# 3dv-casia/PanoVLM

Hardware: AMD Instinct MI355X
Metric: M residual+Jacobian evals/sec (point-to-plane, 64k pts/scan) (higher is better)
Workload: dtype f64

## Files before the change

panovlm_amd/csrc/pvlm_eval.hip:

```cpp
#include <algorithm>
#include <cmath>
#include <limits>

#include "pvlm_functors.h"
#include "pvlm_internal.h"

using namespace pvlm_dev;

#ifndef PVLM_NT_LOADS
#define PVLM_NT_LOADS 1
#endif
#ifndef PVLM_GLOBAL_LOADS
#define PVLM_GLOBAL_LOADS 1
#endif
typedef double pvlm_dbl2 __attribute__((ext_vector_type(2)));
#if PVLM_GLOBAL_LOADS
template <class T> using pvlm_gptr = const __attribute__((address_space(1))) T*;
#else
template <class T> using pvlm_gptr = const T*;
#endif
typedef pvlm_gptr<pvlm_dbl2> pvlm_col_ptr;
#ifndef PVLM_NT_LOADS_MATERIALISE
#define PVLM_NT_LOADS_MATERIALISE 0
#endif
__device__ __forceinline__ const double* at_byte(const double* base, unsigned bytes) {
  return reinterpret_cast<const double*>(reinterpret_cast<const char*>(base) + bytes);
}
template <bool NT>
__device__ __forceinline__ double2 stream_load2(const double* p) {
  pvlm_col_ptr q = (pvlm_col_ptr)(p);
  const pvlm_dbl2 v = NT ? __builtin_nontemporal_load(q) : *q;
  return make_double2(v.x, v.y);
}
struct pvlm_plane_args {
  const uint16_t* idx;
  const int64_t* pair_idx0;
  const int64_t* chunk_plane0;
  const double* tab;
  const double* const* pair_ptab;
  const int* order;
};
template <bool NT>
__device__ __forceinline__ unsigned stream_load_runs(const uint16_t* base, unsigned row) {
  const auto q = (pvlm_gptr<unsigned>)(reinterpret_cast<const char*>(base) + 2u * row);
  return NT ? __builtin_nontemporal_load(q) : *q;
}
template <bool NT>
__device__ __forceinline__ double stream_load1(const double* p) {
  const auto q = (pvlm_gptr<double>)(p);
  return NT ? __builtin_nontemporal_load(q) : *q;
}
template <bool NT>
__device__ __forceinline__ unsigned stream_load_run(const uint16_t* base, unsigned bytes) {
  const auto q = (pvlm_gptr<uint16_t>)(reinterpret_cast<const char*>(base) + (bytes >> 2));
  return NT ? __builtin_nontemporal_load(q) : *q;
}
template <bool NT>
__device__ __forceinline__ unsigned stream_load_word(const uint16_t* base, unsigned bytes) {
  const auto q = (pvlm_gptr<unsigned>)(reinterpret_cast<const char*>(base) + (bytes >> 1));
  return NT ? __builtin_nontemporal_load(q) : *q;
}
__device__ __forceinline__ double table_load(const double* base, unsigned bytes) {
  return *(pvlm_gptr<double>)(reinterpret_cast<const char*>(base) + bytes);
}
#ifndef PVLM_NT_STORES
#define PVLM_NT_STORES 0
#endif
__device__ __forceinline__ void stream_store2(double2* p, double2 v) {
#if PVLM_NT_STORES
  pvlm_dbl2 w; w.x = v.x; w.y = v.y;
  __builtin_nontemporal_store(w, reinterpret_cast<pvlm_dbl2*>(p));
#else
  *p = v;
#endif
}
__device__ __forceinline__ void stream_store1(double* p, double v) {
#if PVLM_NT_STORES
  __builtin_nontemporal_store(v, p);
#else
  *p = v;
#endif
}


#if defined(__HIP_DEVICE_COMPILE__)
#define PVLM_SCHED_FENCE() __builtin_amdgcn_sched_barrier(0)
#else
#define PVLM_SCHED_FENCE() ((void)0)
#endif
#ifndef PVLM_PREFETCH
#define PVLM_PREFETCH -1
#endif
#ifndef PVLM_FUSED_WAVES
#define PVLM_FUSED_WAVES 2
#endif
#ifndef PVLM_FUSED_WAVES_7COL
#define PVLM_FUSED_WAVES_7COL 4
#endif
#ifndef PVLM_FUSED_WAVES_WAVEFORM
#define PVLM_FUSED_WAVES_WAVEFORM 3
#endif

__global__ void k_pose_table(int n, const double* __restrict__ aa, const double* __restrict__ t, double* __restrict__ tab) {
  const int i = blockIdx.x * blockDim.x + threadIdx.x;
  if (i >= n) return;
  const double x = aa[3 * i], y = aa[3 * i + 1], z = aa[3 * i + 2];
  const double th2 = x * x + y * y + z * z;
  double* o = tab + (size_t)i * PVLM_POSE_TAB;
  double R[9];
  if (th2 > 2.220446049250313e-16) {
    const double th = sqrt(th2);
    const double wx = x / th, wy = y / th, wz = z / th;
    const double c = cos(th), s = sin(th), k = 1.0 - c;
    R[0] = c + wx * wx * k;      R[1] = wx * wy * k - wz * s; R[2] = wy * s + wx * wz * k;
    R[3] = wz * s + wx * wy * k; R[4] = c + wy * wy * k;      R[5] = -wx * s + wy * wz * k;
    R[6] = -wy * s + wx * wz * k; R[7] = wx * s + wy * wz * k; R[8] = c + wz * wz * k;
  } else {
    R[0] = 1; R[1] = -z; R[2] = y; R[3] = z; R[4] = 1; R[5] = -x; R[6] = -y; R[7] = x; R[8] = 1;
  }
  double A, B;
  if (th2 > 1e-6) {
    const double th = sqrt(th2);
    A = (1.0 - cos(th)) / th2;
    B = (th - sin(th)) / (th2 * th);
  } else {
    A = 0.5 - th2 * (1.0 / 24.0) + th2 * th2 * (1.0 / 720.0);
    B = (1.0 / 6.0) - th2 * (1.0 / 120.0) + th2 * th2 * (1.0 / 5040.0);
  }
  const double J[9] = {1.0 + B * (x * x - th2), -A * z + B * x * y,       A * y + B * x * z,
                       A * z + B * x * y,       1.0 + B * (y * y - th2), -A * x + B * y * z,
                       -A * y + B * x * z,      A * x + B * y * z,        1.0 + B * (z * z - th2)};
#pragma unroll
  for (int k = 0; k < 9; ++k) { o[k] = R[k]; o[9 + k] = J[k]; }
  o[18] = t[3 * i]; o[19] = t[3 * i + 1]; o[20] = t[3 * i + 2];
}

__global__ void k_pair_table(int P, const int* __restrict__ ref, const int* __restrict__ nei, int n_poses,
                             const double* __restrict__ pose, double* __restrict__ tab) {
  const int p = blockIdx.x * blockDim.x + threadIdx.x;
  if (p >= P) return;
  const int ir = ref[p], in = nei[p];
  double* o = tab + (size_t)p * PVLM_PAIR_TAB;
  if (ir >= n_poses || in >= n_poses) {
    for (int k = 0; k < PVLM_PAIR_TAB; ++k) o[k] = __longlong_as_double(0x7ff8000000000000LL);
    return;
  }
  const double* a = pose + (size_t)ir * PVLM_POSE_TAB;
  const double* b = pose + (size_t)in * PVLM_POSE_TAB;
  double R[9];
#pragma unroll
  for (int i = 0; i < 3; ++i)
#pragma unroll
    for (int j = 0; j < 3; ++j) R[i * 3 + j] = a[i * 3] * b[j * 3] + a[i * 3 + 1] * b[j * 3 + 1] + a[i * 3 + 2] * b[j * 3 + 2];
#pragma unroll
  for (int k = 0; k < 9; ++k) o[k] = R[k];
#pragma unroll
  for (int i = 0; i < 3; ++i) {
    o[9 + i] = a[18 + i] - (R[i * 3] * b[18] + R[i * 3 + 1] * b[19] + R[i * 3 + 2] * b[20]);
    o[12 + i] = a[18 + i];
  }
#pragma unroll
  for (int k = 0; k < 9; ++k) o[15 + k] = a[9 + k];
#pragma unroll
  for (int i = 0; i < 3; ++i)
#pragma unroll
    for (int j = 0; j < 3; ++j) o[24 + i * 3 + j] = -(R[i * 3] * b[9 + j] + R[i * 3 + 1] * b[9 + 3 + j] + R[i * 3 + 2] * b[9 + 6 + j]);
}

struct pvlm_segment {
  int p;
  const double* cols;
  int64_t n_dev;
  int64_t o0;
  int64_t lo, hi;
};
__device__ __forceinline__ pvlm_segment load_segment(int entry, const double* const* __restrict__ pair_cols, const int64_t* __restrict__ pair_stride,
                                                     const int64_t* __restrict__ out_start, const int* __restrict__ blk_pair,
                                                     const int* __restrict__ blk_chunk, int chunk_rows, int64_t row0 = 0) {
  pvlm_segment s;
  s.p = blk_pair[entry];
  s.cols = pair_cols[s.p];
  s.n_dev = pair_stride[s.p];
  s.o0 = out_start[s.p] - row0;
  const int64_t len = out_start[s.p + 1] - out_start[s.p];
  s.lo = (int64_t)blk_chunk[entry] * chunk_rows;
  s.hi = min(len, s.lo + (int64_t)chunk_rows);
  return s;
}

template <int KIND, bool NORM, int NCOLS>
__global__ __launch_bounds__(256) void k_eval_materialise(const double* const* __restrict__ pair_cols,
                                                          const int64_t* __restrict__ pair_stride,
                                                          const int64_t* __restrict__ out_start,
                                                          const int* __restrict__ blk_pair, const int* __restrict__ blk_chunk,
                                                          int chunk_rows, const double* __restrict__ pair_tab, double weight,
                                                          double* __restrict__ r_out, double* __restrict__ J_out, int blk0, int64_t row0) {
  const auto [p, cols, n_dev, o0, lo, hi] = load_segment(blockIdx.x + blk0, pair_cols, pair_stride, out_start, blk_pair, blk_chunk, chunk_rows, row0);
  double T[PVLM_PAIR_TAB];
#pragma unroll
  for (int k = 0; k < PVLM_PAIR_TAB; ++k) T[k] = pair_tab[(size_t)p * PVLM_PAIR_TAB + k];
  __shared__ __attribute__((aligned(16))) double stage[4][128 * 12];
  const int lane = threadIdx.x & 63, wv = threadIdx.x >> 6;
  const double* Jl = T + 15; const double* Mn = T + 24; const double* R = T;
  const int64_t n_it = (hi - lo + 511) / 512;
  for (int64_t it = 0; it < n_it; ++it) {
    const int64_t j = lo + it * 512 + 2 * (int64_t)threadIdx.x;
    if (j < hi) {
      double2 v[NCOLS];
#pragma unroll
      for (int c = 0; c < NCOLS; ++c) v[c] = stream_load2<PVLM_NT_LOADS_MATERIALISE != 0>(cols + (size_t)c * n_dev + j);
#pragma unroll
      for (int h = 0; h < 2; ++h) {
        if (j + h >= hi) break;
        double rec[NCOLS];
#pragma unroll
        for (int c = 0; c < NCOLS; ++c) rec[c] = h ? v[c].y : v[c].x;
        Wrench w;
        eval_wrench<KIND, NORM>(rec, T, weight, w);
        stream_store1(r_out + o0 + j + h, w.r);
        if (J_out) {
          double Jr[12];
#pragma unroll
          for (int k = 0; k < 3; ++k) {
            Jr[k] = w.c[0] * Jl[k] + w.c[1] * Jl[3 + k] + w.c[2] * Jl[6 + k];
            Jr[3 + k] = w.g[k];
            Jr[6 + k] = w.c[0] * Mn[k] + w.c[1] * Mn[3 + k] + w.c[2] * Mn[6 + k];
            Jr[9 + k] = -(w.g[0] * R[k] + w.g[1] * R[3 + k] + w.g[2] * R[6 + k]);
          }
          double2* dst = reinterpret_cast<double2*>(&stage[wv][(2 * lane + h) * 12]);
#pragma unroll
          for (int k = 0; k < 6; ++k) dst[k] = make_double2(Jr[2 * k], Jr[2 * k + 1]);
        }
      }
    }
    if (J_out) {
      __builtin_amdgcn_wave_barrier();
      const int64_t row0 = lo + it * 512 + (int64_t)wv * 128;
      const int64_t rows = min((int64_t)128, hi - row0);
      if (rows > 0) {
        double2* gdst = reinterpret_cast<double2*>(J_out + (size_t)(o0 + row0) * 12);
        const double2* src = reinterpret_cast<const double2*>(&stage[wv][0]);
        const int n2 = (int)rows * 6;
#pragma unroll
        for (int t = 0; t < 12; ++t) {
          const int e = t * 64 + lane;
          if (e < n2) stream_store2(gdst + e, src[e]);
        }
      }
      __builtin_amdgcn_wave_barrier();
    }
  }
}

template <int KIND, bool NORM, int NCOLS, int W>
__global__ __launch_bounds__(256) void k_eval_wrench(const double* const* __restrict__ pair_cols, const int64_t* __restrict__ pair_stride,
                                                     const int64_t* __restrict__ out_start, const int* __restrict__ blk_pair,
                                                     const int* __restrict__ blk_chunk, int chunk_rows, const double* __restrict__ pair_tab,
                                                     double weight, double* __restrict__ w_out, int blk0, int64_t row0) {
  const auto [p, cols, n_dev, o0, lo, hi] = load_segment(blockIdx.x + blk0, pair_cols, pair_stride, out_start, blk_pair, blk_chunk, chunk_rows, row0);
  double T[15];
#pragma unroll
  for (int k = 0; k < 15; ++k) T[k] = pair_tab[(size_t)p * PVLM_PAIR_TAB + k];
  __shared__ double stage[4][128 * W];
  const int lane = threadIdx.x & 63, wv = threadIdx.x >> 6;
  const int64_t n_it = (hi - lo + 511) / 512;
  for (int64_t it = 0; it < n_it; ++it) {
    const int64_t j = lo + it * 512 + 2 * (int64_t)threadIdx.x;
    if (j < hi) {
      double2 v[NCOLS];
#pragma unroll
      for (int c = 0; c < NCOLS; ++c) v[c] = stream_load2<PVLM_NT_LOADS_MATERIALISE != 0>(cols + (size_t)c * n_dev + j);
#pragma unroll
      for (int h = 0; h < 2; ++h) {
        if (j + h >= hi) break;
        double rec[NCOLS];
#pragma unroll
        for (int c = 0; c < NCOLS; ++c) rec[c] = h ? v[c].y : v[c].x;
        Wrench w;
        eval_wrench<KIND, NORM>(rec, T, weight, w);
        double* dst = &stage[wv][(2 * lane + h) * W];
        if (W == 7) { dst[0] = w.r; dst[1] = w.c[0]; dst[2] = w.c[1]; dst[3] = w.c[2]; dst[4] = w.g[0]; dst[5] = w.g[1]; dst[6] = w.g[2]; }
        else { dst[0] = w.r; dst[1] = w.g[0]; dst[2] = w.g[1]; dst[3] = w.g[2]; }
      }
    }
    __builtin_amdgcn_wave_barrier();
    const int64_t r0 = lo + it * 512 + (int64_t)wv * 128;
    const int64_t rows = min((int64_t)128, hi - r0);
    if (rows > 0) {
      double* g = w_out + (size_t)(o0 + r0) * W;
      const int n = (int)rows * W;
#pragma unroll
      for (int t = 0; t < 2 * W; ++t) {
        const int e = t * 64 + lane;
        if (e < n) stream_store1(g + e, stage[wv][e]);
      }
    }
    __builtin_amdgcn_wave_barrier();
  }
}

__device__ __forceinline__ double wave_sum(double x) {
#pragma unroll
  for (int off = 32; off > 0; off >>= 1) x += __shfl_down(x, off, 64);
  return x;
}

#ifndef PVLM_HUBER_SLOT
#define PVLM_HUBER_SLOT 1
#endif

template <bool WEIGHTED>
__device__ __forceinline__ void accumulate_outer(const double (&vv)[6], double r, double rho1, double half_rho, double* acc) {
  int q = 0;
#pragma unroll
  for (int a = 0; a < 6; ++a) {
    const double wa = WEIGHTED ? rho1 * vv[a] : vv[a];
#pragma unroll
    for (int b = a; b < 6; ++b, ++q) acc[q] = fma(wa, vv[b], acc[q]);
    acc[21 + a] = fma(wa, r, acc[21 + a]);
  }
  acc[27] += half_rho;
}

template <int KIND, bool NORM, int NCOLS, int LOSS>
__device__ __forceinline__ void accumulate_row(const double* rec, const double* T, double weight, double loss_a, double a2, double mh_a2, double* acc) {
  Wrench w;
  eval_wrench<KIND, NORM>(rec, T, weight, w);
  const double s = w.r * w.r;
  const double vv[6] = {w.c[0], w.c[1], w.c[2], w.g[0], w.g[1], w.g[2]};
  if (LOSS != PVLM_LOSS_HUBER) { accumulate_outer<false>(vv, w.r, 1.0, 0.5 * s, acc); return; }
  const bool out = s > a2;
  auto general = [&]() {
    const double rr = fabs(w.r);
    const double inv = fast_rcp(out ? rr : 1.0);
    const double rho1 = out ? fmax(std::numeric_limits<double>::min(), loss_a * inv) : 1.0;
    const double half_rho = out ? fma(loss_a, rr, mh_a2) : 0.5 * s;
    accumulate_outer<true>(vv, w.r, rho1, half_rho, acc);
  };
#if PVLM_HUBER_SLOT && defined(__HIP_DEVICE_COMPILE__)
  const unsigned long long outliers = __ballot(out);
  unsigned long long none = outliers;
  asm("" : "+s"(none));
  if (outliers != 0) general();
  if (none == 0) accumulate_outer<false>(vv, w.r, 1.0, 0.5 * s, acc);
#else
  general();
#endif
}

template <int N>
__device__ __forceinline__ double wave_transpose_sum(const double (&a)[N], int lane) {
  static_assert(N <= 32, "at most 32 values");
  double v[32];
#pragma unroll
  for (int k = 0; k < 32; ++k) v[k] = k < N ? a[k] : 0.0;
#pragma unroll
  for (int half = 16; half >= 1; half >>= 1) {
    const bool up = (lane & (2 * half)) != 0;
#pragma unroll
    for (int k = 0; k < half; ++k) {
      const double keep = up ? v[half + k] : v[k];
      const double send = up ? v[k] : v[half + k];
      v[k] = keep + __shfl_xor(send, 2 * half, 64);
    }
  }
  return v[0] + __shfl_xor(v[0], 1, 64);
}

template <int KIND, bool NORM, int NCOLS, int LOSS, bool PR, bool PT, bool ROT>
__global__ __launch_bounds__(256, (NCOLS == 7 ? PVLM_FUSED_WAVES_7COL : PVLM_FUSED_WAVES)) void k_eval_fused(const double* const* __restrict__ pair_cols,
                                                    const int64_t* __restrict__ pair_stride,
                                                    const int64_t* __restrict__ out_start,
                                                    const int* __restrict__ blk_pair, const int* __restrict__ blk_chunk,
                                                    int chunk_rows, const double* __restrict__ pair_tab, double weight,
                                                    double loss_a, double* __restrict__ partials, pvlm_plane_args pr) {
  static_assert(!PR || NCOLS == 7, "plane runs: the 7-column kinds only");
  static_assert(!PT || PR, "the point table: on top of the plane runs only");
  static_assert(!ROT || PR, "rotated halves: the plane-run forms only");
  const int slot = (PT && pr.order) ? pr.order[blockIdx.x] : (int)blockIdx.x;
  if (PT && slot < 0) return;
  constexpr int NS = PR ? 3 : NCOLS;
  const auto [p, cols, n_dev, o0, lo, hi] = load_segment(slot, pair_cols, pair_stride, out_start, blk_pair, blk_chunk, chunk_rows);
  double T[15];
#pragma unroll
  for (int k = 0; k < 15; ++k) T[k] = pair_tab[(size_t)p * PVLM_PAIR_TAB + k];
  double acc[PVLM_PARTIAL];
#pragma unroll
  for (int k = 0; k < PVLM_PARTIAL; ++k) acc[k] = 0.0;
  const double a2 = uniform_sgpr(loss_a * loss_a), mh_a2 = uniform_sgpr(-0.5 * a2);
  constexpr bool kRotate = ROT;
  constexpr bool kPrefetch = !PR && (PVLM_PREFETCH >= 0 ? (PVLM_PREFETCH != 0) : (KIND == PVLM_POINT2PLANE_METER || KIND == PVLM_POINT2LINE_METER));
  const double* colb[NS];
#pragma unroll
  for (int c = 0; c < NS; ++c) colb[c] = PT ? pr.pair_ptab[p] + (size_t)c * PVLM_POINT_TAB_STRIDE : cols + (size_t)c * n_dev + lo;
  const uint16_t* runb = nullptr;
  const double* tabb = nullptr;
  if (PR) { runb = pr.idx + (PT ? 2 : 1) * (pr.pair_idx0[p] + lo); tabb = pr.tab + 4 * pr.chunk_plane0[slot]; }
  const unsigned span = hi > lo ? (unsigned)(hi - lo) : 0u;
  const unsigned span8 = 8u * span, last8 = span8 - 8u;
  unsigned o = 8u * (threadIdx.x + (threadIdx.x & ~63u));
  auto row_at = [&](unsigned bytes) { return min(bytes, last8); };
  double x[2][NS], nx[2][NS];
  double2 pl[2][2];
  unsigned w[2] = {0u, 0u};
  auto load_word = [&](int h, unsigned bytes) {
    if (PT) w[h] = stream_load_word<PVLM_NT_LOADS != 0>(runb, bytes);
    else w[h] = stream_load_run<PVLM_NT_LOADS != 0>(runb, bytes);
  };
  auto load_cols = [&](double (&dst)[NS], unsigned bytes) {
#pragma unroll
    for (int c = 0; c < NS; ++c) dst[c] = stream_load1<PVLM_NT_LOADS != 0>(at_byte(colb[c], bytes));
  };
  auto gather = [&](int h, unsigned bytes) {
    if (PT) {
      const unsigned q = 8u * (w[h] >> 16);
#pragma unroll
      for (int c = 0; c < NS; ++c) x[h][c] = table_load(colb[c], q);
    } else {
      load_cols(x[h], bytes);
    }
    if (PR) {
      const unsigned at = 32u * (w[h] & 0xffffu);
      pl[h][0] = stream_load2<false>(at_byte(tabb, at));
      pl[h][1] = stream_load2<false>(at_byte(tabb, at + 16u));
      PVLM_SCHED_FENCE();
    }
  };
  auto evaluate = [&](int h, unsigned bytes) {
    if (bytes < span8) {
      double rec[NCOLS];
#pragma unroll
      for (int c = 0; c < NS; ++c) rec[c] = x[h][c];
      if (PR) { rec[3] = pl[h][0].x; rec[4] = pl[h][0].y; rec[5] = pl[h][1].x; rec[6] = pl[h][1].y; }
      accumulate_row<KIND, NORM, NCOLS, LOSS>(rec, T, weight, loss_a, a2, mh_a2, acc);
    }
  };
  if (kRotate) {
    if (o < span8) {
      const unsigned ob = row_at(o + 512u);
      load_word(0, o);
      load_word(1, ob);
      gather(0, o);
      load_word(0, row_at(o + 4096u));
      PVLM_SCHED_FENCE();
      gather(1, ob);
      load_word(1, row_at(o + 4608u));
      PVLM_SCHED_FENCE();
    }
    for (; o < span8; o += 4096) {
      evaluate(0, o);
      PVLM_SCHED_FENCE();
      gather(0, row_at(o + 4096u));
      load_word(0, row_at(o + 8192u));
      PVLM_SCHED_FENCE();
      evaluate(1, o + 512u);
      PVLM_SCHED_FENCE();
      gather(1, row_at(o + 4608u));
      load_word(1, row_at(o + 8704u));
      PVLM_SCHED_FENCE();
    }
  } else {
    if (PR && o < span8) { load_word(0, o); load_word(1, row_at(o + 512u)); }
    if (kPrefetch && o < span8) { load_cols(nx[0], o); load_cols(nx[1], row_at(o + 512u)); }
    for (; o < span8; o += 4096) {
      if (kPrefetch) {
#pragma unroll
        for (int c = 0; c < NS; ++c) { x[0][c] = nx[0][c]; x[1][c] = nx[1][c]; }
        load_cols(nx[0], row_at(o + 4096u));
        load_cols(nx[1], row_at(o + 4608u));
      } else {
        gather(0, o);
        gather(1, row_at(o + 512u));
        if (PR) { load_word(0, row_at(o + 4096u)); load_word(1, row_at(o + 4608u)); }
      }
      evaluate(0, o);
      evaluate(1, o + 512u);
    }
  }
  __shared__ double red[4][PVLM_PARTIAL];
  const int lane = threadIdx.x & 63, wv = threadIdx.x >> 6;
  {
    const double s = wave_transpose_sum<PVLM_PARTIAL>(acc, lane);
    if (!(lane & 1) && (lane >> 1) < PVLM_PARTIAL) red[wv][lane >> 1] = s;
  }
  __syncthreads();
  if (threadIdx.x < PVLM_PARTIAL)
    partials[(size_t)slot * PVLM_PARTIAL + threadIdx.x] =
        ((red[0][threadIdx.x] + red[1][threadIdx.x]) + red[2][threadIdx.x]) + red[3][threadIdx.x];
}

template <int KIND, bool NORM, int NCOLS, int LOSS, bool PR>
__global__ __launch_bounds__(256, PVLM_FUSED_WAVES_WAVEFORM) void k_eval_fused_wave(const double* const* __restrict__ pair_cols,
                                                    const int64_t* __restrict__ pair_stride,
                                                    const int64_t* __restrict__ out_start,
                                                    const int* __restrict__ blk_pair, const int* __restrict__ blk_chunk,
                                                    int chunk_rows, int n_units, const double* __restrict__ pair_tab, double weight,
                                                    double loss_a, double* __restrict__ partials, pvlm_plane_args pr) {
  static_assert(!PR || NCOLS == 7, "plane runs: the 7-column kinds only");
  constexpr int NS = PR ? 3 : NCOLS;
  const int unit = __builtin_amdgcn_readfirstlane(blockIdx.x * 4 + (threadIdx.x >> 6)), lane = threadIdx.x & 63;
  if (unit >= n_units) return;
  const auto [p, cols, n_dev, o0, lo, hi] = load_segment(unit, pair_cols, pair_stride, out_start, blk_pair, blk_chunk, chunk_rows);
  double T[15];
#pragma unroll
  for (int k = 0; k < 15; ++k) T[k] = pair_tab[(size_t)p * PVLM_PAIR_TAB + k];
  double acc[PVLM_PARTIAL];
#pragma unroll
  for (int k = 0; k < PVLM_PARTIAL; ++k) acc[k] = 0.0;
  const double a2 = uniform_sgpr(loss_a * loss_a), mh_a2 = uniform_sgpr(-0.5 * a2);
  const double* colb[NS];
#pragma unroll
  for (int c = 0; c < NS; ++c) colb[c] = cols + (size_t)c * n_dev + lo;
  const uint16_t* runb = nullptr;
  const double* tabb = nullptr;
  if (PR) { runb = pr.idx + pr.pair_idx0[p] + lo; tabb = pr.tab + 4 * pr.chunk_plane0[unit]; }
  const unsigned span = hi > lo ? (unsigned)(hi - lo) : 0u;
  unsigned nx_runs = 0;
  if (PR && 2u * lane < span) nx_runs = stream_load_runs<PVLM_NT_LOADS != 0>(runb, 2u * lane);
  for (unsigned j = 2u * lane; j < span; j += 128) {
    double2 v[NS];
#pragma unroll
    for (int c = 0; c < NS; ++c) v[c] = stream_load2<PVLM_NT_LOADS != 0>(at_byte(colb[c], 8u * j));
    double2 pl[2][2];
    if (PR) {
      const unsigned runs = nx_runs;
#pragma unroll
      for (int h = 0; h < 2; ++h) {
        const unsigned at = 32u * (h ? runs >> 16 : runs & 0xffffu);
        pl[h][0] = stream_load2<false>(at_byte(tabb, at));
        pl[h][1] = stream_load2<false>(at_byte(tabb, at + 16u));
      }
      nx_runs = stream_load_runs<PVLM_NT_LOADS != 0>(runb, j + 128 < span ? j + 128 : j);
    }
#pragma unroll
    for (int h = 0; h < 2; ++h) {
      if (j + h >= span) break;
      double rec[NCOLS];
#pragma unroll
      for (int c = 0; c < NS; ++c) rec[c] = h ? v[c].y : v[c].x;
      if (PR) { rec[3] = pl[h][0].x; rec[4] = pl[h][0].y; rec[5] = pl[h][1].x; rec[6] = pl[h][1].y; }
      accumulate_row<KIND, NORM, NCOLS, LOSS>(rec, T, weight, loss_a, a2, mh_a2, acc);
    }
  }
  const double mine = wave_transpose_sum<PVLM_PARTIAL>(acc, lane);
  if (!(lane & 1) && (lane >> 1) < PVLM_PARTIAL) partials[(size_t)unit * PVLM_PARTIAL + (lane >> 1)] = mine;
}

__global__ __launch_bounds__(128) void k_pair_epilogue(int P, const int* __restrict__ pair_blk_start,
                                                       const double* __restrict__ partials,
                                                       const double* __restrict__ pair_tab, double* __restrict__ out) {
  const int p = blockIdx.x;
  __shared__ double S[6][6], gv[6], Dr[6][6], Dn[6][6], cost;
  __shared__ double tot[PVLM_PARTIAL];
  const int t = threadIdx.x;
  if (t < PVLM_PARTIAL) {
    double s = 0.0;
    for (int b = pair_blk_start[p]; b < pair_blk_start[p + 1]; ++b) s += partials[(size_t)b * PVLM_PARTIAL + t];
    tot[t] = s;
  }
  if (t < 36) {
    const int i = t / 6, j = t % 6;
    const double* T = pair_tab + (size_t)p * PVLM_PAIR_TAB;
    double dr = 0.0, dn = 0.0;
    if (i < 3 && j < 3) { dr = T[15 + i * 3 + j]; dn = T[24 + i * 3 + j]; }
    else if (i >= 3 && j >= 3) { dr = (i == j) ? 1.0 : 0.0; dn = -T[(i - 3) * 3 + (j - 3)]; }
    Dr[i][j] = dr; Dn[i][j] = dn;
  }
  __syncthreads();
  if (t < 36) {
    const int i = t / 6, j = t % 6;
    const int a = i < j ? i : j, b = i < j ? j : i;
    S[i][j] = tot[a * 6 - a * (a - 1) / 2 + (b - a)];
  }
  if (t < 6) gv[t] = tot[21 + t];
  if (t == 0) cost = tot[27];
  __syncthreads();
  double* o = out + (size_t)p * PVLM_PAIR_BLOCK;
  if (t < 108) {
    const int blk = t / 36, i = (t % 36) / 6, j = t % 6;
    const double(*L)[6] = (blk == 2) ? Dn : Dr;
    const double(*Rm)[6] = (blk == 0) ? Dr : Dn;
    double s = 0.0;
    for (int a = 0; a < 6; ++a) {
      double u = 0.0;
      for (int b = 0; b < 6; ++b) u += S[a][b] * Rm[b][j];
      s += L[a][i] * u;
    }
    o[t] = s;
  } else if (t < 120) {
    const int i = (t - 108) % 6;
    const double(*L)[6] = (t < 114) ? Dr : Dn;
    double s = 0.0;
    for (int a = 0; a < 6; ++a) s += L[a][i] * gv[a];
    o[t] = s;
  } else if (t == 120) {
    o[120] = cost;
  }
}

__global__ void k_neq_gather(int n_poses, int n_upairs, const int* __restrict__ diag_off, const int* __restrict__ diag_items,
                             const int* __restrict__ off_off, const int* __restrict__ off_items,
                             const double* __restrict__ pair_blocks, int P, int zero_first, double* __restrict__ packed) {
  const int b = blockIdx.x, t = threadIdx.x;
  double* Hd = packed;
  double* Ho = packed + (size_t)n_poses * 36;
  double* g = Ho + (size_t)n_upairs * 36;
  double* cost = g + (size_t)n_poses * 6;
  if (b < n_poses) {
    if (t < 42) {
      double s = 0.0;
      for (int k = diag_off[b]; k < diag_off[b + 1]; ++k) {
        const int it = diag_items[k];
        const double* pb = pair_blocks + (size_t)(it >> 1) * PVLM_PAIR_BLOCK;
        const int role = it & 1;
        s += (t < 36) ? pb[(role ? 72 : 0) + t] : pb[108 + (role ? 6 : 0) + (t - 36)];
      }
      double* dst = (t < 36) ? &Hd[(size_t)b * 36 + t] : &g[(size_t)b * 6 + (t - 36)];
      *dst = zero_first ? s : (*dst + s);
    }
  } else if (b < n_poses + n_upairs) {
    const int u = b - n_poses;
    if (t < 36) {
      const int i = t / 6, j = t % 6;
      double s = 0.0;
      for (int k = off_off[u]; k < off_off[u + 1]; ++k) {
        const int it = off_items[k];
        const double* pb = pair_blocks + (size_t)(it >> 1) * PVLM_PAIR_BLOCK + 36;
        s += (it & 1) ? pb[j * 6 + i] : pb[t];
      }
      double* dst = &Ho[(size_t)u * 36 + t];
      *dst = zero_first ? s : (*dst + s);
    }
  } else {
    __shared__ double red[256];
    double s = 0.0;
    for (int p = t; p < P; p += 256) s += pair_blocks[(size_t)p * PVLM_PAIR_BLOCK + 120];
    red[t] = s;
    __syncthreads();
    for (int w = 128; w > 0; w >>= 1) { if (t < w) red[t] += red[t + w]; __syncthreads(); }
    if (t == 0) *cost = zero_first ? red[0] : (*cost + red[0]);
  }
}

static pvlm_status ensure_pose_cap(pvlm_ctx* ctx, int n) {
  if (n <= ctx->cap_poses) return PVLM_OK;
  if (ctx->capturing) { PVLM_SET_ERR(ctx, "pose table would grow inside a graph capture (run the step once before pvlm_graph_begin)"); return PVLM_ERR_STATE; }
  PVLM_TRY_SYNC(ctx);
  pvlm_i_free(ctx, ctx->d_aa); pvlm_i_free(ctx, ctx->d_t); pvlm_i_free(ctx, ctx->d_pose_tab);
  ctx->d_aa = ctx->d_t = ctx->d_pose_tab = nullptr;
  ctx->cap_poses = 0;
  pvlm_status st;
  if ((st = pvlm_i_alloc(ctx, &ctx->d_aa, (size_t)n * 3))) return st;
  if ((st = pvlm_i_alloc(ctx, &ctx->d_t, (size_t)n * 3))) return st;
  if ((st = pvlm_i_alloc(ctx, &ctx->d_pose_tab, (size_t)n * PVLM_POSE_TAB))) return st;
  ctx->cap_poses = n;
  return PVLM_OK;
}

static pvlm_status pose_table_launch(pvlm_ctx* ctx, int n, const double* d_aa, const double* d_t) {
  if (n > 0) {
    hipLaunchKernelGGL(k_pose_table, dim3((n + 63) / 64), dim3(64), 0, ctx->stream, n, d_aa, d_t, ctx->d_pose_tab);
    PVLM_HIP(ctx, hipGetLastError());
  }
  ctx->n_poses = n;
  ctx->poses_set = true;
  ctx->pose_epoch++;
  return PVLM_OK;
}

static pvlm_status ensure_pair_table(pvlm_ctx* ctx, const pvlm_resset* crs) {
  pvlm_resset* rs = const_cast<pvlm_resset*>(crs);
  if (!ctx->poses_set) { PVLM_SET_ERR(ctx, "pvlm_set_poses must be called before evaluation"); return PVLM_ERR_STATE; }
  for (int p = 0; p < rs->n_pairs; ++p)
    if (rs->h_ref[p] >= ctx->n_poses || rs->h_nei[p] >= ctx->n_poses) {
      PVLM_SET_ERR(ctx, "segment %d references pose %d/%d but only %d poses are set", p, rs->h_ref[p], rs->h_nei[p], ctx->n_poses);
      return PVLM_ERR_STATE;
    }
  if (rs->pair_tab_epoch == ctx->pose_epoch || rs->n_pairs == 0) return PVLM_OK;
  hipLaunchKernelGGL(k_pair_table, dim3((rs->n_pairs + 63) / 64), dim3(64), 0, ctx->stream, rs->n_pairs, rs->d_ref, rs->d_nei,
                     ctx->n_poses, ctx->d_pose_tab, rs->d_pair_tab);
  PVLM_HIP(ctx, hipGetLastError());
  rs->pair_tab_epoch = ctx->pose_epoch;
  return PVLM_OK;
}

template <class K, class... A>
static void launch_eval(K kernel, unsigned grid, pvlm_ctx* ctx, const pvlm_resset* rs, A... rest) {
  hipLaunchKernelGGL(kernel, dim3(grid), dim3(256), 0, ctx->stream, rs->d_pair_cols, rs->d_pair_stride, rs->d_out_start, rs->d_blk_pair, rs->d_blk_chunk,
                     rs->chunk_rows, rest...);
}
template <int KIND, bool NORM, int NCOLS>
static void launch_materialise(pvlm_ctx* ctx, const pvlm_resset* rs, double* d_r, double* d_J, int blk0 = 0, int nblk = -1, int64_t row0 = 0) {
  launch_eval(k_eval_materialise<KIND, NORM, NCOLS>, nblk < 0 ? rs->n_blocks : nblk, ctx, rs, rs->d_pair_tab, rs->weight, d_r, d_J, blk0, row0);
}
template <int KIND, bool NORM, int NCOLS>
static void launch_wrench(pvlm_ctx* ctx, const pvlm_resset* rs, double* d_w, int blk0, int nblk, int64_t row0, bool force_only) {
  launch_eval(force_only ? k_eval_wrench<KIND, NORM, NCOLS, 4> : k_eval_wrench<KIND, NORM, NCOLS, 7>, nblk, ctx, rs, rs->d_pair_tab, rs->weight, d_w, blk0, row0);
}
template <int KIND, bool NORM, int NCOLS, int LOSS, bool PR>
static void launch_fused_as(pvlm_ctx* ctx, const pvlm_resset* rs, double a) {
  const pvlm_plane_args pr = {rs->d_plane_idx, rs->d_pair_idx0, rs->d_chunk_plane0, rs->d_plane_tab, rs->d_pair_ptab, rs->d_order};
  if (rs->wave_units)
    launch_eval(k_eval_fused_wave<KIND, NORM, NCOLS, LOSS, PR>, (rs->n_blocks + 3) / 4, ctx, rs, rs->n_blocks, rs->d_pair_tab, rs->weight, a, rs->d_partials, pr);
  else if (PR && rs->point_table)
    launch_eval(rs->half_rotate ? k_eval_fused<KIND, NORM, NCOLS, LOSS, PR, PR, PR> : k_eval_fused<KIND, NORM, NCOLS, LOSS, PR, PR, false>, rs->n_positions, ctx, rs,
                rs->d_pair_tab, rs->weight, a, rs->d_partials, pr);
  else
    launch_eval(PR && rs->half_rotate ? k_eval_fused<KIND, NORM, NCOLS, LOSS, PR, false, PR> : k_eval_fused<KIND, NORM, NCOLS, LOSS, PR, false, false>, rs->n_blocks, ctx, rs,
                rs->d_pair_tab, rs->weight, a, rs->d_partials, pr);
}
template <int KIND, bool NORM, int NCOLS>
static void launch_fused(pvlm_ctx* ctx, const pvlm_resset* rs, int loss, double a) {
  if constexpr (NCOLS == 7) {
    if (rs->plane_runs) {
      if (loss == PVLM_LOSS_HUBER) launch_fused_as<KIND, NORM, NCOLS, PVLM_LOSS_HUBER, true>(ctx, rs, a);
      else launch_fused_as<KIND, NORM, NCOLS, PVLM_LOSS_NONE, true>(ctx, rs, a);
      return;
    }
  }
  if (loss == PVLM_LOSS_HUBER) launch_fused_as<KIND, NORM, NCOLS, PVLM_LOSS_HUBER, false>(ctx, rs, a);
  else launch_fused_as<KIND, NORM, NCOLS, PVLM_LOSS_NONE, false>(ctx, rs, a);
}

#define PVLM_DISPATCH(FN, ...)                                                                         \
  do {                                                                                                 \
    const bool nz = (rs->flags & PVLM_FLAG_NORMALIZE_DISTANCE) != 0;                                   \
    switch (rs->kind) {                                                                                \
      case PVLM_POINT2PLANE_METER: FN<PVLM_POINT2PLANE_METER, false, 7>(__VA_ARGS__); break;           \
      case PVLM_POINT2PLANE_ANGLE:                                                                     \
        if (nz) FN<PVLM_POINT2PLANE_ANGLE, true, 7>(__VA_ARGS__);                                      \
        else FN<PVLM_POINT2PLANE_ANGLE, false, 7>(__VA_ARGS__);                                        \
        break;                                                                                         \
      case PVLM_POINT2LINE_METER: FN<PVLM_POINT2LINE_METER, false, 9>(__VA_ARGS__); break;             \
      case PVLM_POINT2LINE_ANGLE:                                                                      \
        if (nz) FN<PVLM_POINT2LINE_ANGLE, true, 9>(__VA_ARGS__);                                       \
        else FN<PVLM_POINT2LINE_ANGLE, false, 9>(__VA_ARGS__);                                         \
        break;                                                                                         \
      case PVLM_PLANE2PLANE_GLOBAL: FN<PVLM_PLANE2PLANE_GLOBAL, false, 10>(__VA_ARGS__); break;        \
      case PVLM_PLANE_IOU: FN<PVLM_PLANE_IOU, false, 12>(__VA_ARGS__); break;                          \
    }                                                                                                  \
  } while (0)

extern "C" {

pvlm_status pvlm_set_poses(pvlm_ctx* ctx, int n, const double* aa, const double* t) {
  if (!ctx || n < 0 || (n > 0 && (!aa || !t))) return PVLM_ERR_ARG;
  if (pvlm_i_bind(ctx)) return PVLM_ERR_HIP;
  pvlm_status st = ensure_pose_cap(ctx, n);
  if (st) return st;
  if (n > 0) {
    if ((st = pvlm_i_h2d_q(ctx, ctx->d_aa, aa, (size_t)n * 3 * sizeof(double)))) return st;
    if ((st = pvlm_i_h2d_q(ctx, ctx->d_t, t, (size_t)n * 3 * sizeof(double)))) return st;
  }
  ctx->host_poses_known = false;
  if ((st = pose_table_launch(ctx, n, ctx->d_aa, ctx->d_t))) return st;
  ctx->host_poses.assign(aa, aa + 3 * (size_t)n);
  ctx->host_poses.insert(ctx->host_poses.end(), t, t + 3 * (size_t)n);
  ctx->host_poses_known = true;
  return PVLM_OK;
}

pvlm_status pvlm_set_poses_dev(pvlm_ctx* ctx, int n, const double* d_aa, const double* d_t) {
  if (!ctx || n < 0 || (n > 0 && (!d_aa || !d_t))) return PVLM_ERR_ARG;
  if (pvlm_i_bind(ctx)) return PVLM_ERR_HIP;
  pvlm_status st = ensure_pose_cap(ctx, n);
  if (st) return st;
  ctx->host_poses_known = false;
  return pose_table_launch(ctx, n, d_aa, d_t);
}

pvlm_status pvlm_eval_dev(pvlm_ctx* ctx, const pvlm_resset* rs, double* d_r, double* d_J) {
  if (!ctx || !rs || !d_r) return PVLM_ERR_ARG;
  if (pvlm_i_bind(ctx)) return PVLM_ERR_HIP;
  pvlm_status st = ensure_pair_table(ctx, rs);
  if (st) return st;
  if (rs->n_blocks == 0) return PVLM_OK;
  {
    pvlm_prof_scope prof(ctx, 1);
    PVLM_DISPATCH(launch_materialise, ctx, rs, d_r, d_J);
  }
  PVLM_HIP(ctx, hipGetLastError());
  return PVLM_OK;
}

pvlm_status pvlm_eval(pvlm_ctx* ctx, const pvlm_resset* rs, double* r, double* J) {
  if (!ctx || !rs || (rs->n > 0 && !r)) return PVLM_ERR_ARG;
  if (rs->n == 0) return ensure_pair_table(ctx, rs);
  if (pvlm_i_bind(ctx)) return PVLM_ERR_HIP;
  double *d_r = nullptr, *d_J = nullptr;
  pvlm_status st = pvlm_i_alloc(ctx, &d_r, (size_t)rs->n);
  if (!st && J) st = pvlm_i_alloc(ctx, &d_J, (size_t)rs->n * 12);
  if (!st) st = pvlm_eval_dev(ctx, rs, d_r, d_J);
  if (!st) st = pvlm_i_d2h_q(ctx, r, d_r, (size_t)rs->n * sizeof(double));
  if (!st && J) st = pvlm_i_d2h_q(ctx, J, d_J, (size_t)rs->n * 12 * sizeof(double));
  { const pvlm_status s2 = pvlm_i_sync(ctx); if (!st) st = s2; }
  pvlm_i_free(ctx, d_r); pvlm_i_free(ctx, d_J);
  return st;
}

static pvlm_status eval_to_host(pvlm_ctx* ctx, const pvlm_resset* crs, int mode, double* h_a, double* h_b) {
  pvlm_resset* rs = const_cast<pvlm_resset*>(crs);
  pvlm_status st = ensure_pair_table(ctx, rs);
  if (st) return st;
  if (mode >= 1 && h_b && rs->n_pairs > 0)
    PVLM_HIP(ctx, hipMemcpyAsync(h_b, rs->d_pair_tab, (size_t)rs->n_pairs * PVLM_PAIR_TAB * sizeof(double), hipMemcpyDeviceToHost, ctx->stream));
  if (rs->n == 0) return PVLM_OK;
  int64_t stage_rows = 32ll << 20;
  if (const char* e = getenv("PVLM_STAGE_ROWS")) { const long long v = atoll(e); if (v > 0) stage_rows = v; }
  const int width = mode == 1 ? 7 : (mode == 2 ? 4 : (h_b ? 13 : 1));
  auto slice_end = [&](int p) {
    int q = p + 1;
    while (q < rs->n_pairs && rs->h_out_start[q + 1] - rs->h_out_start[p] <= stage_rows) ++q;
    return q;
  };
  int64_t need = 0;
  for (int p = 0, q; p < rs->n_pairs; p = q) { q = slice_end(p); need = std::max<int64_t>(need, rs->h_out_start[q] - rs->h_out_start[p]); }
  if (rs->stage_doubles < (size_t)need * width) {
    if (ctx->capturing) { PVLM_SET_ERR(ctx, "staging buffer would grow inside a graph capture"); return PVLM_ERR_STATE; }
    pvlm_i_free(ctx, rs->d_stage); rs->d_stage = nullptr; rs->stage_doubles = 0;
    if ((st = pvlm_i_alloc(ctx, &rs->d_stage, (size_t)need * width))) return st;
    rs->stage_doubles = (size_t)need * width;
  }
  for (int p = 0, q; p < rs->n_pairs; p = q) {
    q = slice_end(p);
    const int blk0 = rs->h_pair_blk_start[p], nblk = rs->h_pair_blk_start[q] - blk0;
    const int64_t row0 = rs->h_out_start[p], rows = rs->h_out_start[q] - row0;
    if (nblk > 0) {
      double* d_r = rs->d_stage;
      double* d_J = rs->d_stage + rows;
      {
        pvlm_prof_scope prof(ctx, 1);
        if (mode >= 1) PVLM_DISPATCH(launch_wrench, ctx, rs, rs->d_stage, blk0, nblk, row0, mode == 2);
        else PVLM_DISPATCH(launch_materialise, ctx, rs, d_r, h_b ? d_J : nullptr, blk0, nblk, row0);
      }
      PVLM_HIP(ctx, hipGetLastError());
      if (mode >= 1) PVLM_HIP(ctx, hipMemcpyAsync(h_a + (size_t)row0 * width, rs->d_stage, (size_t)rows * width * sizeof(double), hipMemcpyDeviceToHost, ctx->stream));
      else {
        PVLM_HIP(ctx, hipMemcpyAsync(h_a + row0, d_r, (size_t)rows * sizeof(double), hipMemcpyDeviceToHost, ctx->stream));
        if (h_b) PVLM_HIP(ctx, hipMemcpyAsync(h_b + (size_t)row0 * 12, d_J, (size_t)rows * 12 * sizeof(double), hipMemcpyDeviceToHost, ctx->stream));
      }
    }
  }
  return PVLM_OK;
}

pvlm_status pvlm_eval_host_async(pvlm_ctx* ctx, const pvlm_resset* rs, double* residuals, double* jacobians) {
// ... 198 lines not shown
```

panovlm_amd/csrc/pvlm_functors.h:

```cpp
#pragma once
#include <hip/hip_runtime.h>

#include "pvlm_internal.h"

namespace pvlm_dev {

struct Wrench { double r; double c[3]; double g[3]; };

__device__ __forceinline__ double dot3(const double* a, const double* b) { return a[0] * b[0] + a[1] * b[1] + a[2] * b[2]; }
__device__ __forceinline__ void cross3(const double* a, const double* b, double* o) {
  o[0] = a[1] * b[2] - a[2] * b[1]; o[1] = a[2] * b[0] - a[0] * b[2]; o[2] = a[0] * b[1] - a[1] * b[0];
}


__device__ __forceinline__ double fast_rcp(double x) {
  const double r = __builtin_amdgcn_rcp(x);
  return fma(r, fma(-x, r, 1.0), r);
}
__device__ __forceinline__ double fast_rsqrt(double x) {
  const double r = __builtin_amdgcn_rsq(x);
  return fma(r, fma(-x * r, 0.5 * r, 0.5), r);
}
#ifndef PVLM_ATAN_TIER
#define PVLM_ATAN_TIER 1
#endif
#define PVLM_ATAN_TIER_ENTRY 6
template <int ENTRY = 0>
__device__ __forceinline__ double horner10_sconst(double u, double c0, double c1, double c2, double c3, double c4, double c5, double c6, double c7,
                                                  double c8, double c9) {
  static_assert(ENTRY == 0 || ENTRY == 6, "entry points with a statement below");
#if defined(__HIP_DEVICE_COMPILE__)
  double p;
  if (ENTRY == 6) {
    asm("v_mov_b64 %0, %2\n\t"
        "v_fma_f64 %0, %0, %1, %3\n\t"
        "v_fma_f64 %0, %0, %1, %4\n\t"
        "v_fma_f64 %0, %0, %1, %5\n\t"
        "v_fma_f64 %0, %0, %1, 1.0"
        : "=&v"(p)
        : "v"(u), "s"(c6), "s"(c7), "s"(c8), "s"(c9));
    return p;
  }
  asm("v_mov_b64 %0, %2\n\t"
      "v_fma_f64 %0, %0, %1, %3\n\t"
      "v_fma_f64 %0, %0, %1, %4\n\t"
      "v_fma_f64 %0, %0, %1, %5\n\t"
      "v_fma_f64 %0, %0, %1, %6\n\t"
      "v_fma_f64 %0, %0, %1, %7\n\t"
      "v_fma_f64 %0, %0, %1, %8\n\t"
      "v_fma_f64 %0, %0, %1, %9\n\t"
      "v_fma_f64 %0, %0, %1, %10\n\t"
      "v_fma_f64 %0, %0, %1, %11\n\t"
      "v_fma_f64 %0, %0, %1, 1.0"
      : "=&v"(p)
      : "v"(u), "s"(c0), "s"(c1), "s"(c2), "s"(c3), "s"(c4), "s"(c5), "s"(c6), "s"(c7), "s"(c8), "s"(c9));
  return p;
#else
  const double c[11] = {c0, c1, c2, c3, c4, c5, c6, c7, c8, c9, 1.0};
  double p = c[ENTRY];
  for (int k = ENTRY + 1; k < 11; ++k) p = fma(p, u, c[k]);
  return p;
#endif
}
__device__ __forceinline__ double uniform_sgpr(double x) {
#if defined(__HIP_DEVICE_COMPILE__)
  const unsigned long long b = (unsigned long long)__double_as_longlong(x);
  const unsigned lo = (unsigned)__builtin_amdgcn_readfirstlane((int)(unsigned)b), hi = (unsigned)__builtin_amdgcn_readfirstlane((int)(unsigned)(b >> 32));
  return __longlong_as_double((long long)(((unsigned long long)hi << 32) | lo));
#else
  return x;
#endif
}
template <int ENTRY = 0>
__device__ __forceinline__ double atan_small(double t) {
  const double u = t * t;
  return t * horner10_sconst<ENTRY>(u, 2.11272689568591313e-02, -4.34739031566048761e-02, 5.68812005923421543e-02, -6.64019012732186553e-02,
                                    7.68994845277858746e-02, -9.09077271667437237e-02, 1.11111061650365134e-01, -1.42857141805968924e-01,
                                    1.99999999988503901e-01, -3.33333333333284132e-01);
}
__device__ __forceinline__ double atan2_octants(double y, double x) {
  const double ax = fabs(x);
  const double mn = fmin(y, ax), mx = fmax(y, ax);
  const double a = mn * fast_rcp(mx);
  const bool big = a > 0.41421356237309503;
  const double red = (a - 1.0) * fast_rcp(a + 1.0);
  double r = atan_small(big ? red : a);
  r = big ? r + 0.78539816339744830962 : r;
  r = (y > ax) ? 1.57079632679489661923 - r : r;
  return (x < 0.0) ? 3.14159265358979323846 - r : r;
}
__device__ __forceinline__ double atan2_pos(double y, double x) {
  const bool tiny = PVLM_ATAN_TIER && __all(32.0 * y <= x);
  if (tiny || __all(y <= 0.41421356237309503 * x)) {
    const double t = y * fast_rcp(x);
    return tiny ? atan_small<PVLM_ATAN_TIER_ENTRY>(t) : atan_small(t);
  }
  return atan2_octants(y, x);
}
__device__ __forceinline__ double atan2_pos_grad(double y, double x, bool live, double& inv_h2) {
  const double h2 = fma(x, x, y * y);
  double r;
  const bool tiny = PVLM_ATAN_TIER && __all(32.0 * y <= x);
  if (tiny || __all(y <= 0.41421356237309503 * x)) {
    const double R = live ? fast_rcp(x * h2) : 0.0;
    inv_h2 = x * R;
    const double t = y * (h2 * R);
    r = tiny ? atan_small<PVLM_ATAN_TIER_ENTRY>(t) : atan_small(t);
  } else {
    inv_h2 = live ? fast_rcp(h2) : 0.0;
    r = live ? atan2_octants(y, x) : 0.0;
  }
  return r;
}

__device__ __forceinline__ bool angle_between(const double* v1, const double* v2, double& r, double* g1, double* g2) {
  const double d = dot3(v1, v2);
  const double q1 = dot3(v1, v1), q2 = dot3(v2, v2);
  const double n1 = sqrt(q1), n2 = sqrt(q2);
  const double c = d / (n1 * n2);
  if (c >= 1.0) { r = 0.0; return false; }
  if (c <= -1.0) { r = M_PI; return false; }
  double w[3], a1[3], a2[3];
  cross3(v1, v2, w);
  const double nw = sqrt(dot3(w, w));
  if (!(nw > 0.0)) { r = d < 0.0 ? M_PI : 0.0; return false; }
  r = atan2_pos(nw, d);
  cross3(v1, w, a1);
  cross3(v2, w, a2);
  const double k1 = 1.0 / (q1 * nw), k2 = -1.0 / (q2 * nw);
#pragma unroll
  for (int k = 0; k < 3; ++k) { g1[k] = k1 * a1[k]; g2[k] = k2 * a2[k]; }
  return true;
}

template <bool NORM>
__device__ __forceinline__ bool normalized_angle(const double* P, const double* Pp, double& r, double* gP, double* gPp) {
  if (NORM) {
    const double nu2 = dot3(Pp, Pp);
    const double nu = sqrt(nu2);
    const double ratio = (nu - 1.0) / nu;
    double v1[3], v2[3], g1[3], g2[3];
#pragma unroll
    for (int k = 0; k < 3; ++k) { const double ck = ratio * Pp[k]; v1[k] = Pp[k] - ck; v2[k] = P[k] - ck; }
    if (!angle_between(v1, v2, r, g1, g2)) return false;
    double gc[3] = {-(g1[0] + g2[0]), -(g1[1] + g2[1]), -(g1[2] + g2[2])};
    const double s = dot3(Pp, gc) / (nu2 * nu);
#pragma unroll
    for (int k = 0; k < 3; ++k) { gP[k] = g2[k]; gPp[k] = g1[k] + ratio * gc[k] + s * Pp[k]; }
    return true;
  }
  return angle_between(P, Pp, r, gP, gPp);
}

template <int KIND, bool NORM>
__device__ __forceinline__ void residual_grad(const double* P, const double* rec, double w, double& r, double* g) {
  g[0] = g[1] = g[2] = 0.0;
  r = 0.0;
  if (KIND == PVLM_POINT2PLANE_METER) {
    const double* n = rec + 3;
    const double sd = n[0] * P[0] + n[1] * P[1] + n[2] * P[2] + n[3];
    const double s = sd < 0.0 ? -w : w;
    r = s * sd;
    g[0] = s * n[0]; g[1] = s * n[1]; g[2] = s * n[2];
  } else if (KIND == PVLM_POINT2PLANE_ANGLE && NORM) {
    const double* n = rec + 3;
    const double dd = n[3];
    const double sd = n[0] * P[0] + n[1] * P[1] + n[2] * P[2] + dd;
    const double dis = fabs(sd);
    const double u[3] = {P[0] - (sd - dd) * n[0], P[1] - (sd - dd) * n[1], P[2] - (sd - dd) * n[2]};
    const double q2 = dot3(u, u);
    const double nu2 = q2 + dd * dd;
    const double inv_nu = fast_rsqrt(nu2);
    const double invq = q2 > 0.0 ? fast_rsqrt(q2) : 0.0;
    const double q = q2 * invq, nu = nu2 * inv_nu;
    const double X = fma(-sd, dd, nu), Y = dis * q;
    const bool live = dis >= 1e-3;
    double AD = q * nu, BD = dis * dd * fma(-sd, nu, dd) * (invq * inv_nu);
#if defined(__HIP_DEVICE_COMPILE__)
    asm volatile("" : "+v"(AD), "+v"(BD));
#endif
    double k0;
    r = atan2_pos_grad(Y, X, live, k0);
    const double A = copysign(AD * k0, sd);
    const double B = BD * k0;
#pragma unroll
    for (int k = 0; k < 3; ++k) g[k] = A * n[k] + B * u[k];
  } else if (KIND == PVLM_POINT2PLANE_ANGLE) {
    const double* n = rec + 3;
    const double sd = n[0] * P[0] + n[1] * P[1] + n[2] * P[2] + n[3];
    const double s = sd < 0.0 ? -1.0 : 1.0;
    const double dis = s * sd;
    if (dis < 1e-3) return;
    double Pp[3] = {P[0] - dis * n[0], P[1] - dis * n[1], P[2] - dis * n[2]};
    double sig = 1.0;
    if (fabs(n[0] * Pp[0] + n[1] * Pp[1] + n[2] * Pp[2] + n[3]) > 1e-4) {
      Pp[0] = P[0] + dis * n[0]; Pp[1] = P[1] + dis * n[1]; Pp[2] = P[2] + dis * n[2];
      sig = -1.0;
    }
    double gP[3], gPp[3];
    if (!normalized_angle<NORM>(P, Pp, r, gP, gPp)) return;
    const double t = sig * s * dot3(n, gPp);
#pragma unroll
    for (int k = 0; k < 3; ++k) g[k] = gP[k] + gPp[k] - t * n[k];
  } else if (KIND == PVLM_POINT2LINE_METER) {
    const double* A = rec + 3; const double* d = rec + 6;
    const double dd = d[0] * d[0] + d[1] * d[1] + d[2] * d[2];
    const double k = (d[0] * (P[0] - A[0]) + d[1] * (P[1] - A[1]) + d[2] * (P[2] - A[2])) / dd;
    const double e[3] = {k * d[0] + A[0] - P[0], k * d[1] + A[1] - P[1], k * d[2] + A[2] - P[2]};
    const double dist = sqrt(dot3(e, e));
    r = w * dist;
    const double q = dot3(d, e) / dd;
    const double wi = w / dist;
#pragma unroll
    for (int kk = 0; kk < 3; ++kk) g[kk] = wi * (q * d[kk] - e[kk]);
  } else if (KIND == PVLM_POINT2LINE_ANGLE) {
    const double* A = rec + 3; const double* d = rec + 6;
    const double k = d[0] * (P[0] - A[0]) + d[1] * (P[1] - A[1]) + d[2] * (P[2] - A[2]);
    const double Pp[3] = {k * d[0] + A[0], k * d[1] + A[1], k * d[2] + A[2]};
    const double e[3] = {P[0] - Pp[0], P[1] - Pp[1], P[2] - Pp[2]};
    const double dis = sqrt(dot3(e, e));
    if (dis < 1e-3) return;
    double gP[3], gPp[3];
    if (!normalized_angle<NORM>(P, Pp, r, gP, gPp)) return;
    const double t = dot3(d, gPp);
#pragma unroll
    for (int kk = 0; kk < 3; ++kk) g[kk] = gP[kk] + t * d[kk];
  }
}

template <int KIND, bool NORM>
__device__ __forceinline__ void eval_wrench(const double* rec, const double* T, double w, Wrench& out) {
  const double* R = T; const double* trn = T + 9; const double* trw = T + 12;
  auto chain = [&](const double* p, double* o) {
    o[0] = R[0] * p[0] + R[1] * p[1] + R[2] * p[2] + trn[0];
    o[1] = R[3] * p[0] + R[4] * p[1] + R[5] * p[2] + trn[1];
    o[2] = R[6] * p[0] + R[7] * p[1] + R[8] * p[2] + trn[2];
  };
  if (KIND <= PVLM_POINT2LINE_ANGLE) {
    double P[3];
    chain(rec, P);
    residual_grad<KIND, NORM>(P, rec, w, out.r, out.g);
    const double m[3] = {P[0] - trw[0], P[1] - trw[1], P[2] - trw[2]};
    cross3(m, out.g, out.c);
  } else if (KIND == PVLM_PLANE2PLANE_GLOBAL) {
    const double* ni = rec; const double wk = rec[9];
    double a[3], b[3], nrm[3];
    chain(rec + 3, a);
    chain(rec + 6, b);
    cross3(a, b, nrm);
    out.r = 0.0;
#pragma unroll
    for (int k = 0; k < 3; ++k) { out.c[k] = 0.0; out.g[k] = 0.0; }
    const double dp = dot3(ni, nrm);
    const double s = dp < 0.0 ? -1.0 : 1.0;
    const double q1 = dot3(ni, ni), q2 = dot3(nrm, nrm);
    const double c = s * dp / (sqrt(q1) * sqrt(q2));
    if (c >= 1.0) return;
    double wv[3], nxw[3];
    cross3(ni, nrm, wv);
    const double nw = sqrt(dot3(wv, wv));
    if (!(nw > 0.0)) return;
    out.r = wk * atan2_pos(nw, s * dp);
    cross3(nrm, wv, nxw);
    const double kg = -wk * s / (q2 * nw);
    double gn[3], ga[3], gb[3], ca[3], cb[3];
#pragma unroll
    for (int k = 0; k < 3; ++k) gn[k] = kg * nxw[k];
    cross3(b, gn, ga);
    cross3(gn, a, gb);
    const double ma[3] = {a[0] - trw[0], a[1] - trw[1], a[2] - trw[2]};
    const double mb[3] = {b[0] - trw[0], b[1] - trw[1], b[2] - trw[2]};
    cross3(ma, ga, ca);
    cross3(mb, gb, cb);
#pragma unroll
    for (int k = 0; k < 3; ++k) { out.c[k] = ca[k] + cb[k]; out.g[k] = ga[k] + gb[k]; }
  } else {
    const double* n = rec; const double* mr = rec + 7; const double ang = rec[10]; const double wk = rec[11];
    double mc[3];
    chain(rec + 4, mc);
    out.r = 0.0;
#pragma unroll
    for (int k = 0; k < 3; ++k) { out.c[k] = 0.0; out.g[k] = 0.0; }
    const double sd = n[0] * mc[0] + n[1] * mc[1] + n[2] * mc[2] + n[3];
    const double s = sd < 0.0 ? -1.0 : 1.0;
    const double dis = s * sd;
    double np[3] = {mc[0] - dis * n[0], mc[1] - dis * n[1], mc[2] - dis * n[2]};
    double sig = 1.0;
    if (fabs(n[0] * np[0] + n[1] * np[1] + n[2] * np[2] + n[3]) > 1e-4) {
      np[0] = mc[0] + dis * n[0]; np[1] = mc[1] + dis * n[1]; np[2] = mc[2] + dis * n[2];
      sig = -1.0;
    }
    double cur, g1[3], g2[3];
    const bool smooth = angle_between(np, mr, cur, g1, g2);
    if (cur < ang) return;
    out.r = wk * (cur - ang);
    if (!smooth) return;
    const double t = sig * s * dot3(n, g1);
    double g[3];
#pragma unroll
    for (int k = 0; k < 3; ++k) g[k] = wk * (g1[k] - t * n[k]);
    const double m[3] = {mc[0] - trw[0], mc[1] - trw[1], mc[2] - trw[2]};
    cross3(m, g, out.c);
#pragma unroll
    for (int k = 0; k < 3; ++k) out.g[k] = g[k];
  }
}

}
```

Before: 160,900.

## Accumulate moments about origin and shift normal-equation sums once per lane

Per-row moment vectors are now computed about the world origin rather than the translation point, which removes a vector subtraction per row. Each lane's accumulated 6x6 normal-equation block and gradient are then shifted to the trw reference point algebraically once at the end. For kinds where the moment is orthogonal to the gradient, one cross-term entry is skipped in the per-row loop and rebuilt from the identity c·g = 0 (acc[14] = -(acc[3]+acc[9])). The trade-off is extra end-of-kernel work and possible cancellation error, because the sums accumulate larger lever arms before the shift.

Result: no change. 162,300 (median of 6 runs) (+0.9%).

```diff
diff --git a/panovlm_amd/csrc/pvlm_eval.hip b/panovlm_amd/csrc/pvlm_eval.hip
--- a/panovlm_amd/csrc/pvlm_eval.hip
+++ b/panovlm_amd/csrc/pvlm_eval.hip
@@ -309,40 +309,72 @@
 #define PVLM_HUBER_SLOT 1
 #endif
 
-template <bool WEIGHTED>
+constexpr int kDerivedSum = 14;
+template <bool WEIGHTED, bool DERIVED>
 __device__ __forceinline__ void accumulate_outer(const double (&vv)[6], double r, double rho1, double half_rho, double* acc) {
   int q = 0;
 #pragma unroll
   for (int a = 0; a < 6; ++a) {
     const double wa = WEIGHTED ? rho1 * vv[a] : vv[a];
 #pragma unroll
-    for (int b = a; b < 6; ++b, ++q) acc[q] = fma(wa, vv[b], acc[q]);
+    for (int b = a; b < 6; ++b, ++q)
+      if (!(DERIVED && q == kDerivedSum)) acc[q] = fma(wa, vv[b], acc[q]);
     acc[21 + a] = fma(wa, r, acc[21 + a]);
   }
   acc[27] += half_rho;
 }
 
-template <int KIND, bool NORM, int NCOLS, int LOSS>
+template <int KIND>
+constexpr bool moment_orthogonal = KIND != PVLM_PLANE2PLANE_GLOBAL;
+
+template <bool DERIVED, bool ORIGIN>
+__device__ __forceinline__ void finish_lane_sums(double* acc, const double* t) {
+  auto at = [](int a, int b) { return a <= b ? a * 6 - a * (a - 1) / 2 + (b - a) : b * 6 - b * (b - 1) / 2 + (a - b); };
+  if (DERIVED) acc[kDerivedSum] = 0.0 - (acc[at(0, 3)] + acc[at(1, 4)]);
+  if (!ORIGIN) return;
+  double cg[3][3];
+#pragma unroll
+  for (int i = 0; i < 3; ++i)
+#pragma unroll
+    for (int j = 0; j < 3; ++j)
+      cg[i][j] = fma(t[(i + 2) % 3], acc[at(3 + (i + 1) % 3, 3 + j)], fma(-t[(i + 1) % 3], acc[at(3 + (i + 2) % 3, 3 + j)], acc[at(i, 3 + j)]));
+#pragma unroll
+  for (int i = 0; i < 3; ++i)
+#pragma unroll
+    for (int j = i; j < 3; ++j) {
+      const double k_gc = fma(t[(i + 2) % 3], acc[at(j, 3 + (i + 1) % 3)], fma(-t[(i + 1) % 3], acc[at(j, 3 + (i + 2) % 3)], acc[at(i, j)]));
+      acc[at(i, j)] = fma(t[(j + 2) % 3], cg[i][(j + 1) % 3], fma(-t[(j + 1) % 3], cg[i][(j + 2) % 3], k_gc));
+    }
+#pragma unroll
+  for (int i = 0; i < 3; ++i) {
+#pragma unroll
+    for (int j = 0; j < 3; ++j) acc[at(i, 3 + j)] = cg[i][j];
+    acc[21 + i] = fma(t[(i + 2) % 3], acc[24 + (i + 1) % 3], fma(-t[(i + 1) % 3], acc[24 + (i + 2) % 3], acc[21 + i]));
+  }
+}
+
+template <int KIND, bool NORM, int NCOLS, int LOSS, bool ORIGIN>
 __device__ __forceinline__ void accumulate_row(const double* rec, const double* T, double weight, double loss_a, double a2, double mh_a2, double* acc) {
+  constexpr bool D = moment_orthogonal<KIND>;
   Wrench w;
-  eval_wrench<KIND, NORM>(rec, T, weight, w);
+  eval_wrench<KIND, NORM, ORIGIN>(rec, T, weight, w);
   const double s = w.r * w.r;
   const double vv[6] = {w.c[0], w.c[1], w.c[2], w.g[0], w.g[1], w.g[2]};
-  if (LOSS != PVLM_LOSS_HUBER) { accumulate_outer<false>(vv, w.r, 1.0, 0.5 * s, acc); return; }
+  if (LOSS != PVLM_LOSS_HUBER) { accumulate_outer<false, D>(vv, w.r, 1.0, 0.5 * s, acc); return; }
   const bool out = s > a2;
   auto general = [&]() {
     const double rr = fabs(w.r);
     const double inv = fast_rcp(out ? rr : 1.0);
     const double rho1 = out ? fmax(std::numeric_limits<double>::min(), loss_a * inv) : 1.0;
     const double half_rho = out ? fma(loss_a, rr, mh_a2) : 0.5 * s;
-    accumulate_outer<true>(vv, w.r, rho1, half_rho, acc);
+    accumulate_outer<true, D>(vv, w.r, rho1, half_rho, acc);
   };
 #if PVLM_HUBER_SLOT && defined(__HIP_DEVICE_COMPILE__)
   const unsigned long long outliers = __ballot(out);
   unsigned long long none = outliers;
   asm("" : "+s"(none));
   if (outliers != 0) general();
-  if (none == 0) accumulate_outer<false>(vv, w.r, 1.0, 0.5 * s, acc);
+  if (none == 0) accumulate_outer<false, D>(vv, w.r, 1.0, 0.5 * s, acc);
 #else
   general();
 #endif
@@ -432,7 +464,7 @@
 #pragma unroll
       for (int c = 0; c < NS; ++c) rec[c] = x[h][c];
       if (PR) { rec[3] = pl[h][0].x; rec[4] = pl[h][0].y; rec[5] = pl[h][1].x; rec[6] = pl[h][1].y; }
-      accumulate_row<KIND, NORM, NCOLS, LOSS>(rec, T, weight, loss_a, a2, mh_a2, acc);
+      accumulate_row<KIND, NORM, NCOLS, LOSS, true>(rec, T, weight, loss_a, a2, mh_a2, acc);
     }
   };
   if (kRotate) {
@@ -477,6 +509,7 @@
       evaluate(1, o + 512u);
     }
   }
+  finish_lane_sums<moment_orthogonal<KIND>, true>(acc, T + 12);
   __shared__ double red[4][PVLM_PARTIAL];
   const int lane = threadIdx.x & 63, wv = threadIdx.x >> 6;
   {
@@ -539,9 +572,10 @@
 #pragma unroll
       for (int c = 0; c < NS; ++c) rec[c] = h ? v[c].y : v[c].x;
       if (PR) { rec[3] = pl[h][0].x; rec[4] = pl[h][0].y; rec[5] = pl[h][1].x; rec[6] = pl[h][1].y; }
-      accumulate_row<KIND, NORM, NCOLS, LOSS>(rec, T, weight, loss_a, a2, mh_a2, acc);
-    }
-  }
+      accumulate_row<KIND, NORM, NCOLS, LOSS, true>(rec, T, weight, loss_a, a2, mh_a2, acc);
+    }
+  }
+  finish_lane_sums<moment_orthogonal<KIND>, true>(acc, T + 12);
   const double mine = wave_transpose_sum<PVLM_PARTIAL>(acc, lane);
   if (!(lane & 1) && (lane >> 1) < PVLM_PARTIAL) partials[(size_t)unit * PVLM_PARTIAL + (lane >> 1)] = mine;
 }
diff --git a/panovlm_amd/csrc/pvlm_functors.h b/panovlm_amd/csrc/pvlm_functors.h
--- a/panovlm_amd/csrc/pvlm_functors.h
+++ b/panovlm_amd/csrc/pvlm_functors.h
@@ -228,7 +228,7 @@
   }
 }
 
-template <int KIND, bool NORM>
+template <int KIND, bool NORM, bool ORIGIN = false>
 __device__ __forceinline__ void eval_wrench(const double* rec, const double* T, double w, Wrench& out) {
   const double* R = T; const double* trn = T + 9; const double* trw = T + 12;
   auto chain = [&](const double* p, double* o) {
@@ -240,6 +240,7 @@
     double P[3];
     chain(rec, P);
     residual_grad<KIND, NORM>(P, rec, w, out.r, out.g);
+    if (ORIGIN) { cross3(P, out.g, out.c); return; }
     const double m[3] = {P[0] - trw[0], P[1] - trw[1], P[2] - trw[2]};
     cross3(m, out.g, out.c);
   } else if (KIND == PVLM_PLANE2PLANE_GLOBAL) {
@@ -268,10 +269,15 @@
     for (int k = 0; k < 3; ++k) gn[k] = kg * nxw[k];
     cross3(b, gn, ga);
     cross3(gn, a, gb);
-    const double ma[3] = {a[0] - trw[0], a[1] - trw[1], a[2] - trw[2]};
-    const double mb[3] = {b[0] - trw[0], b[1] - trw[1], b[2] - trw[2]};
-    cross3(ma, ga, ca);
-    cross3(mb, gb, cb);
+    if (ORIGIN) {
+      cross3(a, ga, ca);
+      cross3(b, gb, cb);
+    } else {
+      const double ma[3] = {a[0] - trw[0], a[1] - trw[1], a[2] - trw[2]};
+      const double mb[3] = {b[0] - trw[0], b[1] - trw[1], b[2] - trw[2]};
+      cross3(ma, ga, ca);
+      cross3(mb, gb, cb);
+    }
 #pragma unroll
     for (int k = 0; k < 3; ++k) { out.c[k] = ca[k] + cb[k]; out.g[k] = ga[k] + gb[k]; }
   } else {
@@ -299,8 +305,12 @@
     double g[3];
 #pragma unroll
     for (int k = 0; k < 3; ++k) g[k] = wk * (g1[k] - t * n[k]);
-    const double m[3] = {mc[0] - trw[0], mc[1] - trw[1], mc[2] - trw[2]};
-    cross3(m, g, out.c);
+    if (ORIGIN) {
+      cross3(mc, g, out.c);
+    } else {
+      const double m[3] = {mc[0] - trw[0], mc[1] - trw[1], mc[2] - trw[2]};
+      cross3(m, g, out.c);
+    }
 #pragma unroll
     for (int k = 0; k < 3; ++k) out.g[k] = g[k];
   }
```
